# MooreThreads/LiteGS

Hardware: NVIDIA H100
Metric: forward+backward views/sec @1080p 1M Gaussians (higher is better)
Workload: dtype f32

## Files before the change

### litegs_b200/csrc/common.cuh

```cuda
#pragma once
#include <cuda_runtime.h>
#include <stdint.h>
#include <stdio.h>
#include <type_traits>

#define LGS_OK 0
#define LGS_ERR_ARG 10001
#define LGS_ERR_WORKSPACE 10002

void lgs_set_error(const char* fmt, ...);

#define LGS_REQUIRE(cond, ...)                                   \
    do {                                                         \
        if (!(cond)) {                                           \
            lgs_set_error(__VA_ARGS__);                          \
            return LGS_ERR_ARG;                                  \
        }                                                        \
    } while (0)

#define LGS_CHECK_LAUNCH(what)                                                               \
    do {                                                                                     \
        cudaError_t e__ = cudaGetLastError();                                                \
        if (e__ != cudaSuccess) {                                                            \
            lgs_set_error("%s: %s (%s:%d)", what, cudaGetErrorString(e__), __FILE__, __LINE__); \
// ... 12 lines not shown

static inline int lgs_cdiv(long long a, long long b) { return (int)((a + b - 1) / b); }
static inline bool lgs_tile_ok(int th, int tw)
{
    return (th == 8 && tw == 16) || (th == 12 && tw == 16) || (th == 16 && tw == 16) || (th == 8 && tw == 8);
}

template <typename F> static inline int lgs_with_flags(F&& f) { return f(); }
template <typename F, typename... R> static inline int lgs_with_flags(F&& f, bool b, R... rest)
{
    if (b) return lgs_with_flags([&](auto... c) { return f(std::true_type{}, c...); }, rest...);
    return lgs_with_flags([&](auto... c) { return f(std::false_type{}, c...); }, rest...);
}

template <typename F> static inline int lgs_with_tile(int th, int tw, F&& f)
{
    using I8 = std::integral_constant<int, 8>;
    using I12 = std::integral_constant<int, 12>;
    using I16 = std::integral_constant<int, 16>;
    if (th == 8 && tw == 16) return f(I8{}, I16{});
    if (th == 12 && tw == 16) return f(I12{}, I16{});
    if (th == 16 && tw == 16) return f(I16{}, I16{});
    return f(I8{}, I8{});
}

template <typename F> static inline int lgs_with_degree(int d, F&& f)
{
    switch (d) {
    case 0: return f(std::integral_constant<int, 0>{});
    case 1: return f(std::integral_constant<int, 1>{});
    case 2: return f(std::integral_constant<int, 2>{});
    default: return f(std::integral_constant<int, 3>{});
    }
}

template <auto K> static int lgs_max_threads()
{
    static const int n = [] { cudaFuncAttributes a; return cudaFuncGetAttributes(&a, K) == cudaSuccess ? a.maxThreadsPerBlock : 0; }();
    return n;
}

struct __align__(16) SplatRec {
    float px, py, A, B;
    float C, o, r, g;
    float b, depth, pad0, pad1;
};
static_assert(sizeof(SplatRec) == 48, "SplatRec must be 48 bytes");
#define LGS_REC_FLOATS 12

#define LGS_GRAD_FLOATS 12
#define LGS_GRAD_DEPTH 10
struct LgsRasterGrad { float dmx, dmy, dA, dB, dC, dop; };
#ifdef __CUDACC__
__device__ __forceinline__ void lgs_finish_raster_grad(const float4& a, const float4& c, const float4& e, float A, float B, float C,
                                                       float o, LgsRasterGrad& g)
{
    g.dmx = -(A * a.x + B * a.y);
    g.dmy = -(B * a.x + C * a.y);
    g.dA = -0.5f * a.z;
    g.dB = -a.w;
    g.dC = -0.5f * c.x;
    g.dop = (o > 0.0f) ? e.x / o : 0.0f;
}
#endif
```

### litegs_b200/csrc/raster.cu

```cuda
#include "common.cuh"

#define FULL_MASK 0xffffffffu
#define LOG2E 1.4426950408889634f
#define ALPHA_MIN (1.0f / 256.0f)
#define ALPHA_MAX (255.0f / 256.0f)
#define T_MIN (1.0f / 8192.0f)
#define WARPS_PER_BLOCK 4

__device__ __forceinline__ float fast_ex2(float x)
{
    float y;
    asm("ex2.approx.ftz.f32 %0, %1;" : "=f"(y) : "f"(x));
    return y;
}
__device__ __forceinline__ float fast_rcp(float x)
{
    float y;
    asm("rcp.approx.ftz.f32 %0, %1;" : "=f"(y) : "f"(x));
    return y;
}

__device__ __forceinline__ float2 add2(float2 a, float2 b) { return make_float2(__fadd_rn(a.x, b.x), __fadd_rn(a.y, b.y)); }
__device__ __forceinline__ float2 mul2(float2 a, float2 b) { return make_float2(__fmul_rn(a.x, b.x), __fmul_rn(a.y, b.y)); }
__device__ __forceinline__ float2 fma2(float2 a, float2 b, float2 c) { return make_float2(__fmaf_rn(a.x, b.x, c.x), __fmaf_rn(a.y, b.y, c.y)); }
// ... 31 lines not shown
        "@pk fma.rn.f32 %3, %9, w, %3;\n"
        "@pk fma.rn.f32 %4, %13, w, %4;\n"
        "@pk fma.rn.f32 %0, %12, w, %0;\n"
        "}\n"
        : "+f"(Ts), "+f"(Cr), "+f"(Cg), "+f"(Cb), "+f"(D), "+f"(nf)
        : "f"(a), "f"(cr), "f"(cg), "f"(cb), "f"(ts_min), "f"(a_min), "f"(neg_ki), "f"(z));
}
template <bool DEPTH>
__device__ __forceinline__ void blend_pixel_normal(float a, float cr, float cg, float cb, float z, float n0, float n1, float n2,
                                                   float& Ts, float& Cr, float& Cg, float& Cb, float& D, float& N0, float& N1,
                                                   float& N2, float& nf, float ts_min, float a_min, float neg_ki)
{
    if (DEPTH) {
        asm("{\n"
            ".reg .pred pa, pk;\n"
            ".reg .f32 w;\n"
            "setp.gt.f32 pa, %0, %13;\n"
            "@pa add.f32 %8, %8, 0f3F800000;\n"
            "setp.ge.and.f32 pk, %9, %14, pa;\n"
            "mul.f32 w, %9, %0;\n"
            "@pk fma.rn.f32 %1, %10, w, %1;\n"
            "@pk fma.rn.f32 %2, %11, w, %2;\n"
            "@pk fma.rn.f32 %3, %12, w, %3;\n"
            "@pk fma.rn.f32 %4, %16, w, %4;\n"
            "@pk fma.rn.f32 %5, %17, w, %5;\n"
            "@pk fma.rn.f32 %6, %18, w, %6;\n"
            "@pk fma.rn.f32 %7, %19, w, %7;\n"
            "@pk fma.rn.f32 %0, %15, w, %0;\n"
            "}\n"
            : "+f"(Ts), "+f"(Cr), "+f"(Cg), "+f"(Cb), "+f"(D), "+f"(N0), "+f"(N1), "+f"(N2), "+f"(nf)
            : "f"(a), "f"(cr), "f"(cg), "f"(cb), "f"(ts_min), "f"(a_min), "f"(neg_ki), "f"(z), "f"(n0), "f"(n1), "f"(n2));
    } else {
        asm("{\n"
            ".reg .pred pa, pk;\n"
            ".reg .f32 w;\n"
            "setp.gt.f32 pa, %0, %12;\n"
            "@pa add.f32 %7, %7, 0f3F800000;\n"
            "setp.ge.and.f32 pk, %8, %13, pa;\n"
            "mul.f32 w, %8, %0;\n"
            "@pk fma.rn.f32 %1, %9, w, %1;\n"
            "@pk fma.rn.f32 %2, %10, w, %2;\n"
            "@pk fma.rn.f32 %3, %11, w, %3;\n"
            "@pk fma.rn.f32 %4, %15, w, %4;\n"
            "@pk fma.rn.f32 %5, %16, w, %5;\n"
            "@pk fma.rn.f32 %6, %17, w, %6;\n"
            "@pk fma.rn.f32 %0, %14, w, %0;\n"
            "}\n"
            : "+f"(Ts), "+f"(Cr), "+f"(Cg), "+f"(Cb), "+f"(N0), "+f"(N1), "+f"(N2), "+f"(nf)
            : "f"(a), "f"(cr), "f"(cg), "f"(cb), "f"(ts_min), "f"(a_min), "f"(neg_ki), "f"(n0), "f"(n1), "f"(n2));
    }
    (void)z; (void)D;
}

__device__ __forceinline__ unsigned smem_u32(const void* p) { return (unsigned)__cvta_generic_to_shared(p); }
__device__ __forceinline__ void cp_async16(void* dst, const void* src)
{
    asm volatile("cp.async.cg.shared.global [%0], [%1], 16;\n" ::"r"(smem_u32(dst)), "l"(src));
}
__device__ __forceinline__ void cp_async_commit() { asm volatile("cp.async.commit_group;\n" ::); }
template <int N> __device__ __forceinline__ void cp_async_wait() { asm volatile("cp.async.wait_group %0;\n" ::"n"(N)); }

__device__ __forceinline__ void mbar_init(uint64_t* bar, unsigned count)
{
    asm volatile("mbarrier.init.shared::cta.b64 [%0], %1;\n" ::"r"(smem_u32(bar)), "r"(count));
}
__device__ __forceinline__ void mbar_expect_tx(uint64_t* bar, unsigned bytes)
{
    asm volatile("mbarrier.arrive.expect_tx.shared::cta.b64 _, [%0], %1;\n" ::"r"(smem_u32(bar)), "r"(bytes));
}
__device__ __forceinline__ bool mbar_try_wait(uint64_t* bar, unsigned parity)
{
    unsigned ok;
    asm volatile(
        "{\n"
        ".reg .pred p;\n"
        "mbarrier.try_wait.parity.shared::cta.b64 p, [%1], %2;\n"
        "selp.u32 %0, 1, 0, p;\n"
        "}\n"
        : "=r"(ok)
        : "r"(smem_u32(bar)), "r"(parity)
        : "memory");
    return ok != 0;
}
__device__ __forceinline__ void mbar_wait(uint64_t* bar, unsigned parity)
{
    while (!mbar_try_wait(bar, parity)) {}
}
__device__ __forceinline__ void bulk_g2s(void* dst, const void* src, unsigned bytes, uint64_t* bar)
{
    asm volatile("cp.async.bulk.shared::cluster.global.mbarrier::complete_tx::bytes [%0], [%1], %2, [%3];\n" ::"r"(smem_u32(dst)),
                 "l"(src), "r"(bytes), "r"(smem_u32(bar))
                 : "memory");
}

template <bool BULK>
struct Stager {
    SplatRec* buf;
    uint64_t* bar;
    unsigned phase_bits;
    unsigned pending;
    int lane;
    __device__ __forceinline__ void init(SplatRec* b, uint64_t* m, int ln)
    {
        buf = b; bar = m; lane = ln; phase_bits = 0; pending = 0;
        if (BULK) {
            if (lane == 0) { mbar_init(&bar[0], 1); mbar_init(&bar[1], 1); }
            asm volatile("fence.mbarrier_init.release.cluster;\n" ::);
            __syncwarp();
        }
    }
    template <bool NORMAL = false>
    __device__ __forceinline__ void issue(int which, const SplatRec* __restrict__ recs, int id, const float4* __restrict__ nrec = nullptr,
                                          float4* nbuf = nullptr)
// ... 957 lines not shown
```

### litegs_b200/csrc/sort.cu

```cuda
#include <cub/device/device_radix_sort.cuh>
#include <cub/block/block_scan.cuh>
#include <algorithm>
#include <cstdlib>
#include <cstring>
#include "common.cuh"

namespace {

constexpr int RS_THREADS = 256;
constexpr int RS_WARPS = RS_THREADS / 32;
constexpr int RS_MAXBINS = 256;

int g_sort_impl = -1;
bool g_sort_forced = false;

int sort_impl()
{
    if (g_sort_impl < 0) {
        const char* e = getenv("LGS_SORT");
        g_sort_forced = e != nullptr;
        g_sort_impl = (e != nullptr && strcmp(e, "cub") == 0) ? 0 : 1;
    }
    return g_sort_impl;
}
// ... 140 lines not shown
        for (int j = 0; j < NS; j++) {
            int r = s_cnt[w][d[j]];
#pragma unroll
            for (int q = 0; q < j; q++) r += __popc(mw[q * set_stride + d[j]]);
            own[j] = mw[j * set_stride + d[j]];
            rank[i0 + j] = (unsigned short)(r + __popc(own[j] & lt));
        }
        __syncwarp();
#pragma unroll
        for (int j = 0; j < NS; j++) {
            if ((own[j] >> lane) <= 1u) {
                if (NS == 1) s_cnt[w][d[j]] = (int)rank[i0 + j] + 1;
                else atomicAdd(&s_cnt[w][d[j]], __popc(own[j]));
                mw[j * set_stride + d[j]] = 0u;
            }
        }
        __syncwarp();
    }
    __syncthreads();
    int tot = 0;
#pragma unroll
    for (int k = 0; k < RS_WARPS; k++) { int c = s_cnt[k][t]; s_cnt[k][t] = tot; tot += c; }
    int dbase;
    BlockScan(s_scan).ExclusiveSum(tot, dbase);
#pragma unroll
    for (int k = 0; k < RS_WARPS; k++) s_cnt[k][t] += dbase;
    s_gofs[t] = gdig - dbase;
    __syncthreads();
#pragma unroll
    for (int i = 0; i < IPT; i++) {
        unsigned d = (((unsigned)key[i] - bias) >> shift) & mask;
        int p = s_cnt[w][d] + rank[i];
        s_k[p] = key[i];
        s_v[p] = val[i];
    }
    __syncthreads();
#pragma unroll
    for (int i = 0; i < IPT; i++) {
        int k = i * RS_THREADS + t;
        if (k < nvalid) {
            KeyT kk = s_k[k];
            int dst = s_gofs[(((unsigned)kk - bias) >> shift) & mask] + k;
            kout[dst] = kk;
            vout[dst] = s_v[k];
        }
    }
}

constexpr unsigned LB_AGG = 1u << 30, LB_INC = 2u << 30, LB_MASK = (1u << 30) - 1u;
constexpr int RS_MAXPASS = 4;

struct GhistArgs { int shift[RS_MAXPASS]; int nbins[RS_MAXPASS]; int passes; };

template <typename KeyT, int IPT>
__global__ void __launch_bounds__(RS_THREADS) rs_ghist_kernel(const KeyT* __restrict__ keys, int n, GhistArgs A, int* __restrict__ ghist,
                                                              unsigned bias, const int* __restrict__ n_dev,
                                                              const unsigned* __restrict__ bias_dev)
{
    constexpr int TILE = RS_THREADS * IPT;
    __shared__ int h[RS_MAXPASS][RS_MAXBINS];
    const int t = threadIdx.x;
    if (n_dev != nullptr) n = min(n, max(*n_dev, 0));
    if (bias_dev != nullptr) bias = *bias_dev;
    const int base = blockIdx.x * TILE;
    if (base >= n) return;
    for (int p = 0; p < A.passes; p++) h[p][t] = 0;
    __syncthreads();
#pragma unroll
    for (int i = 0; i < IPT; i++) {
        const int idx = base + i * RS_THREADS + t;
        if (idx < n) {
            const unsigned k = (unsigned)keys[idx] - bias;
            for (int p = 0; p < A.passes; p++) atomicAdd(&h[p][(k >> A.shift[p]) & (unsigned)(A.nbins[p] - 1)], 1);
        }
    }
    __syncthreads();
    for (int p = 0; p < A.passes; p++)
        if (t < A.nbins[p] && h[p][t] != 0) atomicAdd(&ghist[p * RS_MAXBINS + t], h[p][t]);
}

template <typename KeyT, int IPT>
__global__ void __launch_bounds__(RS_THREADS) rs_onesweep_kernel(const KeyT* __restrict__ kin, const unsigned* __restrict__ vin,
                                                                 KeyT* __restrict__ kout, unsigned* __restrict__ vout, int n, int shift,
                                                                 int nbins, const int* __restrict__ ghist ,
                                                                 unsigned* __restrict__ status ,
                                                                 int* __restrict__ ticket, unsigned bias, const int* __restrict__ n_dev,
                                                                 const unsigned* __restrict__ bias_dev)
{
    constexpr int TILE = RS_THREADS * IPT;
    using BlockScan = cub::BlockScan<int, RS_THREADS>;
    __shared__ int s_cnt[RS_WARPS][RS_MAXBINS];
    __shared__ int s_gofs[RS_MAXBINS];
    __shared__ KeyT s_k[TILE];
    __shared__ unsigned s_v[TILE];
    __shared__ int s_tile;
    static_assert(TILE >= RS_WARPS * RS_MAXBINS, "the match slots alias the value staging buffer");
    unsigned (*s_match)[RS_MAXBINS] = reinterpret_cast<unsigned (*)[RS_MAXBINS]>(s_v);
    __shared__ typename BlockScan::TempStorage s_scan;
    const int t = threadIdx.x, lane = t & 31, w = t >> 5;
    if (n_dev != nullptr) n = min(n, max(*n_dev, 0));
    if (bias_dev != nullptr) bias = *bias_dev;
    if (t == 0) s_tile = atomicAdd(ticket, 1);
#pragma unroll
    for (int k = 0; k < RS_WARPS; k++) { s_cnt[k][t] = 0; s_match[k][t] = 0u; }
    __syncthreads();
    const int tile = s_tile;
    const int base = tile * TILE;
    if (base >= n) return;
    const int nvalid = min(TILE, n - base);
    const unsigned mask = (unsigned)nbins - 1u;
    const unsigned lt = lanemask_lt();
    KeyT key[IPT];
    unsigned val[IPT];
    unsigned short rank[IPT];
#pragma unroll
    for (int i = 0; i < IPT; i++) {
        int loc = w * 32 * IPT + i * 32 + lane;
        bool valid = loc < nvalid;
        key[i] = valid ? kin[base + loc] : (KeyT)(bias - 1u);
        val[i] = valid ? vin[base + loc] : 0u;
    }
    int gdig;
    {
        int tot_d = t < nbins ? ghist[t] : 0;
        BlockScan(s_scan).ExclusiveSum(tot_d, gdig);
    }
    __syncthreads();
#pragma unroll
    for (int i = 0; i < IPT; i++) {
        unsigned d = (((unsigned)key[i] - bias) >> shift) & mask;
        atomicOr(&s_match[w][d], 1u << lane);
        __syncwarp();
        unsigned m = s_match[w][d];
        int r = s_cnt[w][d] + __popc(m & lt);
        rank[i] = (unsigned short)r;
        __syncwarp();
        if ((m >> lane) <= 1u) { s_cnt[w][d] = r + 1; s_match[w][d] = 0u; }
        __syncwarp();
    }
    __syncthreads();
    int tot = 0;
#pragma unroll
    for (int k = 0; k < RS_WARPS; k++) { int c = s_cnt[k][t]; s_cnt[k][t] = tot; tot += c; }
    int real = tot;
    if (t == (int)mask) real -= (TILE - nvalid);
    if (t < nbins) {
        volatile unsigned* st_ = status + (size_t)tile * nbins;
        st_[t] = LB_AGG | (unsigned)real;
        unsigned prefix = 0u;
        for (int i = tile - 1; i >= 0;) {
            const unsigned v = *((volatile unsigned*)(status + (size_t)i * nbins + t));
            const unsigned flag = v & ~LB_MASK;
            if (flag == 0u) continue;
            prefix += v & LB_MASK;
            if (flag == LB_INC) break;
            i--;
        }
        st_[t] = LB_INC | (prefix + (unsigned)real);
        gdig += (int)prefix;
    }
    int dbase;
    BlockScan(s_scan).ExclusiveSum(tot, dbase);
#pragma unroll
    for (int k = 0; k < RS_WARPS; k++) s_cnt[k][t] += dbase;
    s_gofs[t] = gdig - dbase;
    __syncthreads();
#pragma unroll
    for (int i = 0; i < IPT; i++) {
        unsigned d = (((unsigned)key[i] - bias) >> shift) & mask;
        int p = s_cnt[w][d] + rank[i];
        s_k[p] = key[i];
        s_v[p] = val[i];
    }
    __syncthreads();
#pragma unroll
    for (int i = 0; i < IPT; i++) {
        int k = i * RS_THREADS + t;
        if (k < nvalid) {
            KeyT kk = s_k[k];
            int dst = s_gofs[(((unsigned)kk - bias) >> shift) & mask] + k;
            kout[dst] = kk;
            vout[dst] = s_v[k];
        }
    }
}

struct RsPlan {
    int ipt, tile, nblocks, passes, dbits;
    size_t table_bytes, scan_bytes, total_bytes, off_scan, off_keys, off_vals;
};

inline size_t align256(size_t x) { return (x + 255) & ~(size_t)255; }

template <typename KeyT>
RsPlan rs_plan(int n, int begin_bit, int end_bit)
{
    RsPlan p;
    static const int forced_ipt = getenv("LGS_RS_IPT") ? atoi(getenv("LGS_RS_IPT")) : 0;
    p.ipt = (forced_ipt == 8 || forced_ipt == 16) ? forced_ipt : (n > (1 << 22) ? 16 : 8);
    p.tile = RS_THREADS * p.ipt;
    p.nblocks = (n + p.tile - 1) / p.tile;
    int bits = end_bit - begin_bit;
    p.passes = bits <= 0 ? 0 : (bits + 7) / 8;
    p.dbits = p.passes == 0 ? 0 : (bits + p.passes - 1) / p.passes;
    p.table_bytes = align256((size_t)RS_MAXPASS * RS_MAXBINS * p.nblocks * sizeof(int));
    p.scan_bytes = align256((RS_MAXPASS * RS_MAXBINS + 64) * sizeof(int));
    p.off_scan = p.table_bytes;
    p.off_keys = p.off_scan + p.scan_bytes;
    p.off_vals = p.off_keys + align256((size_t)n * sizeof(KeyT));
    p.total_bytes = p.off_vals + align256((size_t)n * sizeof(unsigned));
    return p;
}

bool rs_use_onesweep();
template <typename KeyT>
int rs_sort_onesweep(const KeyT* keys_in, KeyT* keys_out, const unsigned* vals_in, unsigned* vals_out, int n, int begin_bit, int end_bit,
                     unsigned bias, char* ws, cudaStream_t st, const int* n_dev, const unsigned* bias_dev);

template <typename KeyT>
int rs_sort(const KeyT* keys_in, KeyT* keys_out, const unsigned* vals_in, unsigned* vals_out, int n, int begin_bit, int end_bit,
            unsigned bias, char* ws, cudaStream_t st, const int* n_dev = nullptr, const unsigned* bias_dev = nullptr)
{
    RsPlan p = rs_plan<KeyT>(n, begin_bit, end_bit);
    if (p.passes == 0) {
        LGS_REQUIRE(n_dev == nullptr, "sort_pairs: a device-side count needs at least one pass");
        LGS_CUDA(cudaMemcpyAsync(keys_out, keys_in, (size_t)n * sizeof(KeyT), cudaMemcpyDeviceToDevice, st));
        LGS_CUDA(cudaMemcpyAsync(vals_out, vals_in, (size_t)n * sizeof(unsigned), cudaMemcpyDeviceToDevice, st));
        return LGS_OK;
    }
    if (rs_use_onesweep())
        return rs_sort_onesweep<KeyT>(keys_in, keys_out, vals_in, vals_out, n, begin_bit, end_bit, bias, ws, st, n_dev, bias_dev);
    int* table = (int*)ws;
    int* totals = (int*)(ws + p.off_scan);
    KeyT* ktmp = (KeyT*)(ws + p.off_keys);
    unsigned* vtmp = (unsigned*)(ws + p.off_vals);
    const KeyT* ksrc = keys_in;
    const unsigned* vsrc = vals_in;
    int bit = begin_bit;
    for (int pass = 0; pass < p.passes; pass++) {
        int dbits = min(p.dbits, end_bit - bit);
        int nbins = 1 << dbits;
        bool to_out = ((p.passes - 1 - pass) & 1) == 0;
        KeyT* kdst = to_out ? keys_out : ktmp;
        unsigned* vdst = to_out ? vals_out : vtmp;
        const bool vec = ((uintptr_t)ksrc & 15) == 0;
        lgs_with_flags([&](auto ipt16, auto v) {
            rs_hist_kernel<KeyT, ipt16 ? 16 : 8, v><<<p.nblocks, RS_THREADS, 0, st>>>(ksrc, n, bit, nbins, p.nblocks, table, bias, n_dev,
                                                                                     bias_dev);
            return LGS_OK;
        }, p.ipt == 16, vec);
        LGS_CHECK_LAUNCH("rs_hist_kernel");
        rs_scan_rows_kernel<<<nbins, RS_THREADS, 0, st>>>(table, p.nblocks, totals);
        LGS_CHECK_LAUNCH("rs_scan_rows_kernel");
        static const int rank_cap = getenv("LGS_RS_RANK") ? atoi(getenv("LGS_RS_RANK")) : 2;
        int ns = 1;
        while (ns < 4 && ns * 2 <= rank_cap && ns * 2 * RS_WARPS * nbins <= p.tile) ns *= 2;
        lgs_with_flags([&](auto ipt16, auto ns4, auto ns2) {
            rs_scatter_kernel<KeyT, ipt16 ? 16 : 8, ns4 ? 4 : ns2 ? 2 : 1><<<p.nblocks, RS_THREADS, 0, st>>>(
                ksrc, vsrc, kdst, vdst, n, bit, nbins, p.nblocks, table, totals, bias, n_dev, bias_dev);
            return LGS_OK;
        }, p.ipt == 16, ns == 4, ns == 2);
        LGS_CHECK_LAUNCH("rs_scatter_kernel");
        ksrc = kdst; vsrc = vdst;
        bit += dbits;
    }
    return LGS_OK;
}

int g_rs_onesweep = -1;
bool rs_use_onesweep()
{
    if (g_rs_onesweep < 0) {
        const char* e = getenv("LGS_RS");
        g_rs_onesweep = (e != nullptr && e[0] == 'o') ? 1 : 0;
    }
    return g_rs_onesweep == 1;
}

template <typename KeyT>
int rs_sort_onesweep(const KeyT* keys_in, KeyT* keys_out, const unsigned* vals_in, unsigned* vals_out, int n, int begin_bit, int end_bit,
                     unsigned bias, char* ws, cudaStream_t st, const int* n_dev, const unsigned* bias_dev)
{
    RsPlan p = rs_plan<KeyT>(n, begin_bit, end_bit);
    unsigned* status = (unsigned*)ws;
    int* ghist = (int*)(ws + p.off_scan);
    int* tickets = ghist + RS_MAXPASS * RS_MAXBINS;
    KeyT* ktmp = (KeyT*)(ws + p.off_keys);
    unsigned* vtmp = (unsigned*)(ws + p.off_vals);
    GhistArgs A;
    A.passes = p.passes;
    size_t status_words = 0;
    int bit = begin_bit;
    for (int pass = 0; pass < p.passes; pass++) {
        int dbits = min(p.dbits, end_bit - bit);
        A.shift[pass] = bit; A.nbins[pass] = 1 << dbits;
        status_words += (size_t)p.nblocks * A.nbins[pass];
        bit += dbits;
    }
    LGS_CUDA(cudaMemsetAsync(status, 0, status_words * sizeof(unsigned), st));
    LGS_CUDA(cudaMemsetAsync(ghist, 0, (RS_MAXPASS * RS_MAXBINS + 64) * sizeof(int), st));
    lgs_with_flags([&](auto ipt16) {
        rs_ghist_kernel<KeyT, ipt16 ? 16 : 8><<<p.nblocks, RS_THREADS, 0, st>>>(keys_in, n, A, ghist, bias, n_dev, bias_dev);
        return LGS_OK;
    }, p.ipt == 16);
    LGS_CHECK_LAUNCH("rs_ghist_kernel");
    const KeyT* ksrc = keys_in;
    const unsigned* vsrc = vals_in;
    size_t soff = 0;
    for (int pass = 0; pass < p.passes; pass++) {
        bool to_out = ((p.passes - 1 - pass) & 1) == 0;
        KeyT* kdst = to_out ? keys_out : ktmp;
        unsigned* vdst = to_out ? vals_out : vtmp;
        lgs_with_flags([&](auto ipt16) {
            rs_onesweep_kernel<KeyT, ipt16 ? 16 : 8><<<p.nblocks, RS_THREADS, 0, st>>>(ksrc, vsrc, kdst, vdst, n, A.shift[pass],
                A.nbins[pass], ghist + pass * RS_MAXBINS, status + soff, tickets + pass, bias, n_dev, bias_dev);
            return LGS_OK;
        }, p.ipt == 16);
        LGS_CHECK_LAUNCH("rs_onesweep_kernel");
        soff += (size_t)p.nblocks * A.nbins[pass];
        ksrc = kdst; vsrc = vdst;
    }
    return LGS_OK;
}

template <typename KeyT>
size_t sort_workspace_bytes(int n, int max_bits)
{
    size_t cubb = 0;
    cub::DeviceRadixSort::SortPairs<KeyT, unsigned>(nullptr, cubb, nullptr, nullptr, nullptr, nullptr, n, 0, max_bits);
    size_t own = rs_plan<KeyT>(n, 0, max_bits).total_bytes;
    return std::max(cubb, own) + 256;
}

template <typename KeyT>
int sort_pairs(const char* who, const KeyT* keys_in, KeyT* keys_out, const unsigned* vals_in, unsigned* vals_out, int n, int begin_bit,
               int end_bit, unsigned bias, void* workspace, size_t workspace_bytes, void* stream)
{
    if (n <= 0) return LGS_OK;
    LGS_REQUIRE(begin_bit >= 0 && end_bit >= begin_bit && end_bit <= (int)(8 * sizeof(KeyT)), "%s: bad bit range [%d, %d)", who, begin_bit,
                end_bit);
    char* ws = (char*)(((uintptr_t)workspace + 255) & ~(uintptr_t)255);
    size_t need;
    const int impl = sort_impl_for(n, end_bit - begin_bit, bias);
    if (impl == 0) {
        if (bias != 0u) { begin_bit = 0; end_bit = 8 * (int)sizeof(KeyT); }
        need = 0;
        cub::DeviceRadixSort::SortPairs<KeyT, unsigned>(nullptr, need, nullptr, nullptr, nullptr, nullptr, n, begin_bit, end_bit);
    } else {
        need = rs_plan<KeyT>(n, begin_bit, end_bit).total_bytes;
    }
    if (workspace == nullptr || workspace_bytes < need + 256) {
        lgs_set_error("%s: workspace of %zu bytes needed, %zu given", who, need + 256, workspace_bytes);
        return LGS_ERR_WORKSPACE;
    }
    if (impl == 0) {
        LGS_CUDA(cub::DeviceRadixSort::SortPairs<KeyT, unsigned>(ws, need, keys_in, keys_out, vals_in, vals_out, n, begin_bit, end_bit,
                                                                 (cudaStream_t)stream));
        return LGS_OK;
    }
    return rs_sort<KeyT>(keys_in, keys_out, vals_in, vals_out, n, begin_bit, end_bit, bias, ws, (cudaStream_t)stream);
}

}

extern "C" int lgs_set_sort_impl(int impl)
{
    LGS_REQUIRE(impl == -1 || impl == 0 || impl == 1, "set_sort_impl: %d is not -1 (unforced), 0 (cub) or 1 (lgs)", impl);
    g_sort_impl = impl;
    g_sort_forced = impl >= 0;
    return LGS_OK;
}

// ... 87 lines not shown
```

### profiles/microbench/dev_count_bench.py

```python
import ctypes
import sys, os
sys.path.insert(0, os.path.dirname(os.path.dirname(os.path.dirname(os.path.abspath(__file__)))))
import torch
from litegs_b200 import _lib

dev = torch.device("cuda:0")
st = lambda: torch.cuda.current_stream().cuda_stream
P = lambda t: t.data_ptr()


def timeit(fn, n=30):
    for _ in range(5):
        fn()
    torch.cuda.synchronize()
    e0 = torch.cuda.Event(enable_timing=True); e1 = torch.cuda.Event(enable_timing=True)
    e0.record()
    for _ in range(n):
        fn()
    e1.record(); torch.cuda.synchronize()
    return e0.elapsed_time(e1) / n * 1000.0


D = 10_897_674
for cap in (D, int(D * 1.3) + 65536):
    keys = torch.randint(1, 16201, (cap,), device=dev, dtype=torch.int32).to(torch.int16)
    vals = torch.arange(cap, device=dev, dtype=torch.int32)
    ko, vo = torch.empty_like(keys), torch.empty_like(vals)
    nb = ctypes.c_size_t(0)
    _lib.call("lgs_sort_pairs_u16_workspace_bytes", cap, ctypes.byref(nb))
    ws = torch.empty(nb.value, dtype=torch.uint8, device=dev)
    ndev = torch.tensor([D], dtype=torch.int32, device=dev)
    t_host = timeit(lambda: _lib.call("lgs_sort_pairs_u16", P(keys), P(ko), P(vals), P(vo), D, 0, 14, P(ws), ctypes.c_size_t(nb.value), st()))
    t_dev = timeit(lambda: _lib.call("lgs_sort_pairs_u16_dev", P(keys), P(ko), P(vals), P(vo), cap, P(ndev), 0, 14, P(ws), ctypes.c_size_t(nb.value), st()))
    print(f"tile sort D={D} capacity={cap}: host count {t_host:.1f} us, device count {t_dev:.1f} us")

N = 1_000_064
k32 = torch.randint(0, 1 << 24, (N,), device=dev, dtype=torch.int32)
v32 = torch.arange(N, device=dev, dtype=torch.int32)
ko, vo = torch.empty_like(k32), torch.empty_like(v32)
nb = ctypes.c_size_t(0)
_lib.call("lgs_sort_pairs_u32_workspace_bytes", N, ctypes.byref(nb))
ws = torch.empty(nb.value, dtype=torch.uint8, device=dev)
ndev = torch.tensor([984_960], dtype=torch.int32, device=dev)
bias = torch.zeros(1, dtype=torch.int32, device=dev)
t_host = timeit(lambda: _lib.call("lgs_sort_pairs_u32_rebased", P(k32), P(ko), P(v32), P(vo), 984_960, 0, 24, P(ws), ctypes.c_size_t(nb.value), st()))
t_dev = timeit(lambda: _lib.call("lgs_sort_pairs_u32_dev", P(k32), P(ko), P(v32), P(vo), N, P(ndev), P(bias), 24, P(ws), ctypes.c_size_t(nb.value), st()))
print(f"depth sort N=984960 (capacity {N}): host count {t_host:.1f} us, device count {t_dev:.1f} us")
cnt = torch.randint(0, 20, (N,), device=dev, dtype=torch.int32)
out = torch.empty(N, dtype=torch.int32, device=dev)
nb2 = ctypes.c_size_t(0)
_lib.call("lgs_scan_gathered_workspace_bytes", N, ctypes.byref(nb2))
ws2 = torch.empty(nb2.value, dtype=torch.uint8, device=dev)
order = torch.randperm(N, device=dev).to(torch.int32)
t_host = timeit(lambda: _lib.call("lgs_scan_gathered", P(cnt), P(order), 984_960, P(out), P(ws2), ctypes.c_size_t(nb2.value), st()))
t_dev = timeit(lambda: _lib.call("lgs_scan_gathered_dev", P(cnt), P(order), N, P(ndev), P(out), P(ws2), ctypes.c_size_t(nb2.value), st()))
print(f"gathered scan: host count {t_host:.1f} us, device count {t_dev:.1f} us")

D4 = 71_700_532
keys = torch.randint(1, 64801, (D4,), device=dev, dtype=torch.int32).to(torch.int16)
vals = torch.arange(D4, device=dev, dtype=torch.int32)
ko, vo = torch.empty_like(keys), torch.empty_like(vals)
nb = ctypes.c_size_t(0)
_lib.call("lgs_sort_pairs_u16_workspace_bytes", D4, ctypes.byref(nb))
ws = torch.empty(nb.value, dtype=torch.uint8, device=dev)
t = timeit(lambda: _lib.call("lgs_sort_pairs_u16", P(keys), P(ko), P(vals), P(vo), D4, 0, 16, P(ws), ctypes.c_size_t(nb.value), st()), n=10)
print(f"C4 tile sort D={D4}, 16 bits, LGS_RS_IPT={os.environ.get('LGS_RS_IPT', 'default')}, LGS_SORT={os.environ.get('LGS_SORT', 'lgs')}: {t:.1f} us "
      f"= {D4 * (2 + 2 * 12) / t / 1e6:.2f} TB/s of algorithmic traffic")
```

Baseline: 955.0.

## Rework onesweep radix sort with persistent tiles, cp.async staging, and windowed lookback

```diff
diff --git a/litegs_b200/csrc/common.cuh b/litegs_b200/csrc/common.cuh
--- a/litegs_b200/csrc/common.cuh
+++ b/litegs_b200/csrc/common.cuh
@@ -88,6 +88,14 @@
 #define LGS_GRAD_DEPTH 10
 struct LgsRasterGrad { float dmx, dmy, dA, dB, dC, dop; };
 #ifdef __CUDACC__
+__device__ __forceinline__ unsigned smem_u32(const void* p) { return (unsigned)__cvta_generic_to_shared(p); }
+__device__ __forceinline__ void cp_async16(void* dst, const void* src)
+{
+    asm volatile("cp.async.cg.shared.global [%0], [%1], 16;\n" ::"r"(smem_u32(dst)), "l"(src));
+}
+__device__ __forceinline__ void cp_async_commit() { asm volatile("cp.async.commit_group;\n" ::); }
+template <int N> __device__ __forceinline__ void cp_async_wait() { asm volatile("cp.async.wait_group %0;\n" ::"n"(N)); }
+
 __device__ __forceinline__ void lgs_finish_raster_grad(const float4& a, const float4& c, const float4& e, float A, float B, float C,
                                                        float o, LgsRasterGrad& g)
 {
diff --git a/litegs_b200/csrc/raster.cu b/litegs_b200/csrc/raster.cu
--- a/litegs_b200/csrc/raster.cu
+++ b/litegs_b200/csrc/raster.cu
@@ -107,13 +107,6 @@
     (void)z; (void)D;
 }
 
-__device__ __forceinline__ unsigned smem_u32(const void* p) { return (unsigned)__cvta_generic_to_shared(p); }
-__device__ __forceinline__ void cp_async16(void* dst, const void* src)
-{
-    asm volatile("cp.async.cg.shared.global [%0], [%1], 16;\n" ::"r"(smem_u32(dst)), "l"(src));
-}
-__device__ __forceinline__ void cp_async_commit() { asm volatile("cp.async.commit_group;\n" ::); }
-template <int N> __device__ __forceinline__ void cp_async_wait() { asm volatile("cp.async.wait_group %0;\n" ::"n"(N)); }
 
 __device__ __forceinline__ void mbar_init(uint64_t* bar, unsigned count)
 {
diff --git a/litegs_b200/csrc/sort.cu b/litegs_b200/csrc/sort.cu
--- a/litegs_b200/csrc/sort.cu
+++ b/litegs_b200/csrc/sort.cu
@@ -216,142 +216,212 @@
 
 struct GhistArgs { int shift[RS_MAXPASS]; int nbins[RS_MAXPASS]; int passes; };
 
-template <typename KeyT, int IPT>
+template <typename KeyT>
 __global__ void __launch_bounds__(RS_THREADS) rs_ghist_kernel(const KeyT* __restrict__ keys, int n, GhistArgs A, int* __restrict__ ghist,
                                                               unsigned bias, const int* __restrict__ n_dev,
                                                               const unsigned* __restrict__ bias_dev)
 {
-    constexpr int TILE = RS_THREADS * IPT;
+    constexpr int KPV = 16 / (int)sizeof(KeyT);
     __shared__ int h[RS_MAXPASS][RS_MAXBINS];
     const int t = threadIdx.x;
     if (n_dev != nullptr) n = min(n, max(*n_dev, 0));
     if (bias_dev != nullptr) bias = *bias_dev;
-    const int base = blockIdx.x * TILE;
-    if (base >= n) return;
-    for (int p = 0; p < A.passes; p++) h[p][t] = 0;
-    __syncthreads();
-#pragma unroll
-    for (int i = 0; i < IPT; i++) {
-        const int idx = base + i * RS_THREADS + t;
-        if (idx < n) {
-            const unsigned k = (unsigned)keys[idx] - bias;
-            for (int p = 0; p < A.passes; p++) atomicAdd(&h[p][(k >> A.shift[p]) & (unsigned)(A.nbins[p] - 1)], 1);
-        }
-    }
+#pragma unroll
+    for (int p = 0; p < RS_MAXPASS; p++) h[p][t] = 0;
+    __syncthreads();
+    auto count = [&](unsigned key) {
+        const unsigned k = key - bias;
+#pragma unroll
+        for (int p = 0; p < RS_MAXPASS; p++)
+            if (p < A.passes) atomicAdd(&h[p][(k >> A.shift[p]) & (unsigned)(A.nbins[p] - 1)], 1);
+    };
+    const int stride = gridDim.x * RS_THREADS;
+    int done = 0;
+    if (((uintptr_t)keys & 15) == 0) {
+        const int nv = n / KPV;
+        const uint4* v = reinterpret_cast<const uint4*>(keys);
+        for (int i = blockIdx.x * RS_THREADS + t; i < nv; i += stride) {
+            const uint4 q = v[i];
+            const unsigned x[4] = { q.x, q.y, q.z, q.w };
+#pragma unroll
+            for (int c = 0; c < 4; c++) {
+                if (sizeof(KeyT) == 2) { count(x[c] & 0xffffu); count(x[c] >> 16); }
+                else count(x[c]);
+            }
+        }
+        done = nv * KPV;
+    }
+    for (int i = done + blockIdx.x * RS_THREADS + t; i < n; i += stride) count((unsigned)keys[i]);
     __syncthreads();
     for (int p = 0; p < A.passes; p++)
         if (t < A.nbins[p] && h[p][t] != 0) atomicAdd(&ghist[p * RS_MAXBINS + t], h[p][t]);
 }
 
-template <typename KeyT, int IPT>
-__global__ void __launch_bounds__(RS_THREADS) rs_onesweep_kernel(const KeyT* __restrict__ kin, const unsigned* __restrict__ vin,
-                                                                 KeyT* __restrict__ kout, unsigned* __restrict__ vout, int n, int shift,
-                                                                 int nbins, const int* __restrict__ ghist ,
-                                                                 unsigned* __restrict__ status ,
-                                                                 int* __restrict__ ticket, unsigned bias, const int* __restrict__ n_dev,
-                                                                 const unsigned* __restrict__ bias_dev)
-{
-    constexpr int TILE = RS_THREADS * IPT;
-    using BlockScan = cub::BlockScan<int, RS_THREADS>;
-    __shared__ int s_cnt[RS_WARPS][RS_MAXBINS];
+constexpr int LB_WIN = 8;
+
+template <typename KeyT, int NT, int IPT>
+__global__ void __launch_bounds__(NT) rs_onesweep_kernel(const KeyT* __restrict__ kin, const unsigned* __restrict__ vin,
+                                                         KeyT* __restrict__ kout, unsigned* __restrict__ vout, int n, int shift,
+                                                         int nbins, const int* __restrict__ ghist ,
+                                                         unsigned* __restrict__ status ,
+                                                         int* __restrict__ ticket, unsigned bias, const int* __restrict__ n_dev,
+                                                         const unsigned* __restrict__ bias_dev)
+{
+    constexpr int NW = NT / 32, TILE = NT * IPT, NS = 2 * NW * RS_MAXBINS <= TILE ? 2 : 1;
+    static_assert(NT >= RS_MAXBINS, "thread t owns digit t in the block-wide steps");
+    static_assert(IPT % NS == 0 && NS * NW * RS_MAXBINS <= TILE, "the match slots of a round fit in the value staging buffer");
+    static_assert(TILE * sizeof(KeyT) % (16 * NT) == 0, "the staged keys are whole 16-byte copies of every thread");
+    using BlockScan = cub::BlockScan<int, NT>;
+    extern __shared__ __align__(16) unsigned char s_dyn[];
+    unsigned* s_v = reinterpret_cast<unsigned*>(s_dyn);
+    KeyT* s_k = reinterpret_cast<KeyT*>(s_v + TILE);
+    unsigned* s_match = s_v;
+    __shared__ int s_cnt[NW][RS_MAXBINS];
     __shared__ int s_gofs[RS_MAXBINS];
-    __shared__ KeyT s_k[TILE];
-    __shared__ unsigned s_v[TILE];
+    __shared__ int s_gdig[RS_MAXBINS];
+    __shared__ typename BlockScan::TempStorage s_scan;
     __shared__ int s_tile;
-    static_assert(TILE >= RS_WARPS * RS_MAXBINS, "the match slots alias the value staging buffer");
-    unsigned (*s_match)[RS_MAXBINS] = reinterpret_cast<unsigned (*)[RS_MAXBINS]>(s_v);
-    __shared__ typename BlockScan::TempStorage s_scan;
     const int t = threadIdx.x, lane = t & 31, w = t >> 5;
     if (n_dev != nullptr) n = min(n, max(*n_dev, 0));
     if (bias_dev != nullptr) bias = *bias_dev;
-    if (t == 0) s_tile = atomicAdd(ticket, 1);
-#pragma unroll
-    for (int k = 0; k < RS_WARPS; k++) { s_cnt[k][t] = 0; s_match[k][t] = 0u; }
-    __syncthreads();
-    const int tile = s_tile;
-    const int base = tile * TILE;
-    if (base >= n) return;
-    const int nvalid = min(TILE, n - base);
     const unsigned mask = (unsigned)nbins - 1u;
     const unsigned lt = lanemask_lt();
-    KeyT key[IPT];
-    unsigned val[IPT];
-    unsigned short rank[IPT];
-#pragma unroll
-    for (int i = 0; i < IPT; i++) {
-        int loc = w * 32 * IPT + i * 32 + lane;
-        bool valid = loc < nvalid;
-        key[i] = valid ? kin[base + loc] : (KeyT)(bias - 1u);
-        val[i] = valid ? vin[base + loc] : 0u;
-    }
-    int gdig;
+    const bool aligned = (((uintptr_t)kin | (uintptr_t)vin) & 15) == 0;
     {
-        int tot_d = t < nbins ? ghist[t] : 0;
-        BlockScan(s_scan).ExclusiveSum(tot_d, gdig);
-    }
-    __syncthreads();
-#pragma unroll
-    for (int i = 0; i < IPT; i++) {
-        unsigned d = (((unsigned)key[i] - bias) >> shift) & mask;
-        atomicOr(&s_match[w][d], 1u << lane);
-        __syncwarp();
-        unsigned m = s_match[w][d];
-        int r = s_cnt[w][d] + __popc(m & lt);
-        rank[i] = (unsigned short)r;
-        __syncwarp();
-        if ((m >> lane) <= 1u) { s_cnt[w][d] = r + 1; s_match[w][d] = 0u; }
-        __syncwarp();
-    }
-    __syncthreads();
-    int tot = 0;
-#pragma unroll
-    for (int k = 0; k < RS_WARPS; k++) { int c = s_cnt[k][t]; s_cnt[k][t] = tot; tot += c; }
-    int real = tot;
-    if (t == (int)mask) real -= (TILE - nvalid);
-    if (t < nbins) {
-        volatile unsigned* st_ = status + (size_t)tile * nbins;
-        st_[t] = LB_AGG | (unsigned)real;
-        unsigned prefix = 0u;
-        for (int i = tile - 1; i >= 0;) {
-            const unsigned v = *((volatile unsigned*)(status + (size_t)i * nbins + t));
-            const unsigned flag = v & ~LB_MASK;
-            if (flag == 0u) continue;
-            prefix += v & LB_MASK;
-            if (flag == LB_INC) break;
-            i--;
-        }
-        st_[t] = LB_INC | (prefix + (unsigned)real);
-        gdig += (int)prefix;
-    }
-    int dbase;
-    BlockScan(s_scan).ExclusiveSum(tot, dbase);
-#pragma unroll
-    for (int k = 0; k < RS_WARPS; k++) s_cnt[k][t] += dbase;
-    s_gofs[t] = gdig - dbase;
-    __syncthreads();
-#pragma unroll
-    for (int i = 0; i < IPT; i++) {
-        unsigned d = (((unsigned)key[i] - bias) >> shift) & mask;
-        int p = s_cnt[w][d] + rank[i];
-        s_k[p] = key[i];
-        s_v[p] = val[i];
-    }
-    __syncthreads();
-#pragma unroll
-    for (int i = 0; i < IPT; i++) {
-        int k = i * RS_THREADS + t;
-        if (k < nvalid) {
-            KeyT kk = s_k[k];
-            int dst = s_gofs[(((unsigned)kk - bias) >> shift) & mask] + k;
-            kout[dst] = kk;
-            vout[dst] = s_v[k];
-        }
+        int g;
+        BlockScan(s_scan).ExclusiveSum(t < nbins ? ghist[t] : 0, g);
+        if (t < RS_MAXBINS) s_gdig[t] = g;
+    }
+    if (t == 0) s_tile = atomicAdd(ticket, 1);
+    __syncthreads();
+    for (int tile = s_tile; (long long)tile * TILE < n; tile = s_tile) {
+        const int base = tile * TILE;
+        const int nvalid = min(TILE, n - base);
+        const bool staged = aligned && nvalid == TILE;
+        if (staged) {
+            const char* gv = reinterpret_cast<const char*>(vin + base);
+            const char* gk = reinterpret_cast<const char*>(kin + base);
+            for (int c = t * 16; c < TILE * 4; c += NT * 16) cp_async16(s_dyn + c, gv + c);
+            for (int c = t * 16; c < TILE * (int)sizeof(KeyT); c += NT * 16) cp_async16(s_dyn + TILE * 4 + c, gk + c);
+            cp_async_commit();
+            cp_async_wait<0>();
+            __syncthreads();
+        }
+        KeyT key[IPT];
+        unsigned val[IPT];
+        unsigned short rank[IPT];
+#pragma unroll
+        for (int i = 0; i < IPT; i++) {
+            int loc = w * 32 * IPT + i * 32 + lane;
+            if (staged) {
+                key[i] = s_k[loc];
+                val[i] = s_v[loc];
+            } else {
+                bool valid = loc < nvalid;
+                key[i] = valid ? kin[base + loc] : (KeyT)(bias - 1u);
+                val[i] = valid ? vin[base + loc] : 0u;
+            }
+        }
+        if (staged) __syncthreads();
+        for (int k = t; k < NW * RS_MAXBINS; k += NT) (&s_cnt[0][0])[k] = 0;
+        for (int k = t; k < NS * NW * nbins; k += NT) s_match[k] = 0u;
+        __syncthreads();
+        unsigned* mw = s_match + w * nbins;
+        const int set_stride = NW * nbins;
+#pragma unroll
+        for (int i0 = 0; i0 < IPT; i0 += NS) {
+            unsigned d[NS];
+#pragma unroll
+            for (int q = 0; q < NS; q++) {
+                d[q] = (((unsigned)key[i0 + q] - bias) >> shift) & mask;
+                atomicOr(&mw[q * set_stride + d[q]], 1u << lane);
+            }
+            __syncwarp();
+            unsigned own[NS];
+#pragma unroll
+            for (int j = 0; j < NS; j++) {
+                int r = s_cnt[w][d[j]];
+#pragma unroll
+                for (int q = 0; q < j; q++) r += __popc(mw[q * set_stride + d[j]]);
+                own[j] = mw[j * set_stride + d[j]];
+                rank[i0 + j] = (unsigned short)(r + __popc(own[j] & lt));
+            }
+            __syncwarp();
+#pragma unroll
+            for (int j = 0; j < NS; j++) {
+                if ((own[j] >> lane) <= 1u) {
+                    atomicAdd(&s_cnt[w][d[j]], __popc(own[j]));
+                    mw[j * set_stride + d[j]] = 0u;
+                }
+            }
+            __syncwarp();
+        }
+        __syncthreads();
+        int tot = 0;
+        if (t < RS_MAXBINS) {
+#pragma unroll
+            for (int k = 0; k < NW; k++) { int c = s_cnt[k][t]; s_cnt[k][t] = tot; tot += c; }
+        }
+        unsigned* st_ = status + (size_t)tile * nbins;
+        int real = 0;
+        if (t < nbins) {
+            real = tot - (t == (int)mask ? TILE - nvalid : 0);
+            *((volatile unsigned*)&st_[t]) = (tile == 0 ? LB_INC : LB_AGG) | (unsigned)real;
+        }
+        int dbase;
+        BlockScan(s_scan).ExclusiveSum(tot, dbase);
+        if (t < RS_MAXBINS) {
+#pragma unroll
+            for (int k = 0; k < NW; k++) s_cnt[k][t] += dbase;
+        }
+        __syncthreads();
+#pragma unroll
+        for (int i = 0; i < IPT; i++) {
+            unsigned d = (((unsigned)key[i] - bias) >> shift) & mask;
+            int p = s_cnt[w][d] + rank[i];
+            s_k[p] = key[i];
+            s_v[p] = val[i];
+        }
+        if (t < nbins) {
+            unsigned prefix = 0u;
+            for (int j = tile - 1; j >= 0;) {
+                unsigned v[LB_WIN];
+#pragma unroll
+                for (int k = 0; k < LB_WIN; k++)
+                    v[k] = j - k >= 0 ? *((const volatile unsigned*)&status[(size_t)(j - k) * nbins + t]) : LB_INC;
+                int used = 0;
+                bool inc = false;
+#pragma unroll
+                for (int k = 0; k < LB_WIN; k++) {
+                    const unsigned flag = v[k] & ~LB_MASK;
+                    if (used == k && !inc && flag != 0u) { prefix += v[k] & LB_MASK; used++; inc = flag == LB_INC; }
+                }
+                if (inc) break;
+                if (used == 0) __nanosleep(256);
+                j -= used;
+            }
+            if (tile > 0) *((volatile unsigned*)&st_[t]) = LB_INC | (prefix + (unsigned)real);
+            s_gofs[t] = s_gdig[t] + (int)prefix - dbase;
+        }
+        __syncthreads();
+#pragma unroll
+        for (int i = 0; i < IPT; i++) {
+            int k = i * NT + t;
+            if (k < nvalid) {
+                KeyT kk = s_k[k];
+                int dst = s_gofs[(((unsigned)kk - bias) >> shift) & mask] + k;
+                kout[dst] = kk;
+                vout[dst] = s_v[k];
+            }
+        }
+        if (t == 0) s_tile = atomicAdd(ticket, 1);
+        __syncthreads();
     }
 }
 
 struct RsPlan {
     int ipt, tile, nblocks, passes, dbits;
-    size_t table_bytes, scan_bytes, total_bytes, off_scan, off_keys, off_vals;
+    size_t table_bytes, scan_bytes, total_bytes, off_scan, off_table, off_keys, off_vals;
 };
 
 inline size_t align256(size_t x) { return (x + 255) & ~(size_t)255; }
@@ -360,8 +430,7 @@
 RsPlan rs_plan(int n, int begin_bit, int end_bit)
 {
     RsPlan p;
-    static const int forced_ipt = getenv("LGS_RS_IPT") ? atoi(getenv("LGS_RS_IPT")) : 0;
-    p.ipt = (forced_ipt == 8 || forced_ipt == 16) ? forced_ipt : (n > (1 << 22) ? 16 : 8);
+    p.ipt = n > (1 << 22) ? 16 : 8;
     p.tile = RS_THREADS * p.ipt;
     p.nblocks = (n + p.tile - 1) / p.tile;
     int bits = end_bit - begin_bit;
@@ -369,8 +438,9 @@
     p.dbits = p.passes == 0 ? 0 : (bits + p.passes - 1) / p.passes;
     p.table_bytes = align256((size_t)RS_MAXPASS * RS_MAXBINS * p.nblocks * sizeof(int));
     p.scan_bytes = align256((RS_MAXPASS * RS_MAXBINS + 64) * sizeof(int));
-    p.off_scan = p.table_bytes;
-    p.off_keys = p.off_scan + p.scan_bytes;
+    p.off_scan = 0;
+    p.off_table = p.scan_bytes;
+    p.off_keys = p.off_table + p.table_bytes;
     p.off_vals = p.off_keys + align256((size_t)n * sizeof(KeyT));
     p.total_bytes = p.off_vals + align256((size_t)n * sizeof(unsigned));
     return p;
@@ -394,7 +464,7 @@
     }
     if (rs_use_onesweep())
         return rs_sort_onesweep<KeyT>(keys_in, keys_out, vals_in, vals_out, n, begin_bit, end_bit, bias, ws, st, n_dev, bias_dev);
-    int* table = (int*)ws;
+    int* table = (int*)(ws + p.off_table);
     int* totals = (int*)(ws + p.off_scan);
     KeyT* ktmp = (KeyT*)(ws + p.off_keys);
     unsigned* vtmp = (unsigned*)(ws + p.off_vals);
@@ -416,14 +486,12 @@
         LGS_CHECK_LAUNCH("rs_hist_kernel");
         rs_scan_rows_kernel<<<nbins, RS_THREADS, 0, st>>>(table, p.nblocks, totals);
         LGS_CHECK_LAUNCH("rs_scan_rows_kernel");
-        static const int rank_cap = getenv("LGS_RS_RANK") ? atoi(getenv("LGS_RS_RANK")) : 2;
-        int ns = 1;
-        while (ns < 4 && ns * 2 <= rank_cap && ns * 2 * RS_WARPS * nbins <= p.tile) ns *= 2;
-        lgs_with_flags([&](auto ipt16, auto ns4, auto ns2) {
-            rs_scatter_kernel<KeyT, ipt16 ? 16 : 8, ns4 ? 4 : ns2 ? 2 : 1><<<p.nblocks, RS_THREADS, 0, st>>>(
+        const bool ns2 = 2 * RS_WARPS * nbins <= p.tile;
+        lgs_with_flags([&](auto ipt16, auto two) {
+            rs_scatter_kernel<KeyT, ipt16 ? 16 : 8, two ? 2 : 1><<<p.nblocks, RS_THREADS, 0, st>>>(
                 ksrc, vsrc, kdst, vdst, n, bit, nbins, p.nblocks, table, totals, bias, n_dev, bias_dev);
             return LGS_OK;
-        }, p.ipt == 16, ns == 4, ns == 2);
+        }, p.ipt == 16, ns2);
         LGS_CHECK_LAUNCH("rs_scatter_kernel");
         ksrc = kdst; vsrc = vdst;
         bit += dbits;
@@ -436,19 +504,46 @@
 {
     if (g_rs_onesweep < 0) {
         const char* e = getenv("LGS_RS");
-        g_rs_onesweep = (e != nullptr && e[0] == 'o') ? 1 : 0;
+        g_rs_onesweep = (e != nullptr && e[0] == 'p') ? 0 : 1;
     }
     return g_rs_onesweep == 1;
 }
+
+template <typename KeyT, int NT, int IPT>
+int rs_onesweep_pass(const KeyT* ksrc, const unsigned* vsrc, KeyT* kdst, unsigned* vdst, int n, int shift, int nbins, const int* ghist,
+                     unsigned* status, int* ticket, unsigned bias, cudaStream_t st, const int* n_dev, const unsigned* bias_dev, int sms)
+{
+    constexpr int TILE = NT * IPT;
+    constexpr int smem = TILE * (int)(sizeof(unsigned) + sizeof(KeyT));
+    auto kern = rs_onesweep_kernel<KeyT, NT, IPT>;
+    static const int resident = [&] {
+        int b = 0;
+        if (cudaFuncSetAttribute(kern, cudaFuncAttributeMaxDynamicSharedMemorySize, smem) != cudaSuccess ||
+            cudaOccupancyMaxActiveBlocksPerMultiprocessor(&b, kern, NT, smem) != cudaSuccess) return 0;
+        return b;
+    }();
+    LGS_REQUIRE(resident > 0, "rs_onesweep_kernel: no CTA of %d threads and %d bytes of shared memory fits an SM", NT, smem);
+    const int grid = std::min((n + TILE - 1) / TILE, resident * sms);
+    kern<<<grid, NT, smem, st>>>(ksrc, vsrc, kdst, vdst, n, shift, nbins, ghist, status, ticket, bias, n_dev, bias_dev);
+    LGS_CHECK_LAUNCH("rs_onesweep_kernel");
+    return LGS_OK;
+}
+
+template <typename KeyT> struct RsOnesweepShape { static constexpr int NT = 256, IPT = 16; };
+template <> struct RsOnesweepShape<unsigned short> { static constexpr int NT = 512, IPT = 24; };
+
+
 
 template <typename KeyT>
 int rs_sort_onesweep(const KeyT* keys_in, KeyT* keys_out, const unsigned* vals_in, unsigned* vals_out, int n, int begin_bit, int end_bit,
                      unsigned bias, char* ws, cudaStream_t st, const int* n_dev, const unsigned* bias_dev)
 {
     RsPlan p = rs_plan<KeyT>(n, begin_bit, end_bit);
-    unsigned* status = (unsigned*)ws;
+    using S = RsOnesweepShape<KeyT>;
+    const int ntiles = (n + S::NT * S::IPT - 1) / (S::NT * S::IPT);
     int* ghist = (int*)(ws + p.off_scan);
     int* tickets = ghist + RS_MAXPASS * RS_MAXBINS;
+    unsigned* status = (unsigned*)(ws + p.off_table);
     KeyT* ktmp = (KeyT*)(ws + p.off_keys);
     unsigned* vtmp = (unsigned*)(ws + p.off_vals);
     GhistArgs A;
@@ -458,15 +553,15 @@
     for (int pass = 0; pass < p.passes; pass++) {
         int dbits = min(p.dbits, end_bit - bit);
         A.shift[pass] = bit; A.nbins[pass] = 1 << dbits;
-        status_words += (size_t)p.nblocks * A.nbins[pass];
+        status_words += (size_t)ntiles * A.nbins[pass];
         bit += dbits;
     }
-    LGS_CUDA(cudaMemsetAsync(status, 0, status_words * sizeof(unsigned), st));
-    LGS_CUDA(cudaMemsetAsync(ghist, 0, (RS_MAXPASS * RS_MAXBINS + 64) * sizeof(int), st));
-    lgs_with_flags([&](auto ipt16) {
-        rs_ghist_kernel<KeyT, ipt16 ? 16 : 8><<<p.nblocks, RS_THREADS, 0, st>>>(keys_in, n, A, ghist, bias, n_dev, bias_dev);
-        return LGS_OK;
-    }, p.ipt == 16);
+    LGS_CUDA(cudaMemsetAsync(ws, 0, p.off_table + status_words * sizeof(unsigned), st));
+    int dev = 0, sms = 0;
+    LGS_CUDA(cudaGetDevice(&dev));
+    LGS_CUDA(cudaDeviceGetAttribute(&sms, cudaDevAttrMultiProcessorCount, dev));
+    rs_ghist_kernel<KeyT><<<std::min((n + RS_THREADS * 16 - 1) / (RS_THREADS * 16), 8 * sms), RS_THREADS, 0, st>>>(keys_in, n, A, ghist,
+                                                                                                                   bias, n_dev, bias_dev);
     LGS_CHECK_LAUNCH("rs_ghist_kernel");
     const KeyT* ksrc = keys_in;
     const unsigned* vsrc = vals_in;
@@ -475,13 +570,11 @@
         bool to_out = ((p.passes - 1 - pass) & 1) == 0;
         KeyT* kdst = to_out ? keys_out : ktmp;
         unsigned* vdst = to_out ? vals_out : vtmp;
-        lgs_with_flags([&](auto ipt16) {
-            rs_onesweep_kernel<KeyT, ipt16 ? 16 : 8><<<p.nblocks, RS_THREADS, 0, st>>>(ksrc, vsrc, kdst, vdst, n, A.shift[pass],
-                A.nbins[pass], ghist + pass * RS_MAXBINS, status + soff, tickets + pass, bias, n_dev, bias_dev);
-            return LGS_OK;
-        }, p.ipt == 16);
-        LGS_CHECK_LAUNCH("rs_onesweep_kernel");
-        soff += (size_t)p.nblocks * A.nbins[pass];
+        const int rc = rs_onesweep_pass<KeyT, S::NT, S::IPT>(ksrc, vsrc, kdst, vdst, n, A.shift[pass], A.nbins[pass],
+                                                             ghist + pass * RS_MAXBINS, status + soff, tickets + pass, bias, st, n_dev,
+                                                             bias_dev, sms);
+        if (rc != LGS_OK) return rc;
+        soff += (size_t)ntiles * A.nbins[pass];
         ksrc = kdst; vsrc = vdst;
     }
     return LGS_OK;
diff --git a/profiles/microbench/binning_bench.py b/profiles/microbench/binning_bench.py
--- /dev/null
+++ b/profiles/microbench/binning_bench.py
@@ -0,0 +1,160 @@
+import argparse
+import ctypes
+import json
+import os
+import subprocess
+import sys
+
+sys.path.insert(0, os.path.dirname(os.path.dirname(os.path.dirname(os.path.abspath(__file__)))))
+import torch
+
+from litegs_b200 import _lib, pipeline, scene
+from litegs_b200.dist import PARAM_ORDER
+
+ap = argparse.ArgumentParser()
+ap.add_argument("--out", default=None, metavar="DIR", help="also write the results to DIR/binning_bench.json")
+ap.add_argument("--iters", type=int, default=50)
+ap.add_argument("--no-c4", action="store_true")
+args = ap.parse_args()
+
+dev = torch.device("cuda:0")
+P = lambda t: ctypes.c_void_p(t.data_ptr())
+st = lambda: ctypes.c_void_p(torch.cuda.current_stream().cuda_stream)
+FORMS = {"passes": 0, "onesweep": 1}
+
+
+def card():
+    try:
+        q = subprocess.run(["nvidia-smi", "--query-gpu=name,power.limit,clocks.max.sm", "--format=csv,noheader"], capture_output=True,
+                           text=True, timeout=30).stdout.strip().splitlines()[0]
+    except Exception as e:
+        q = f"nvidia-smi unavailable: {e}"
+    return f"{torch.cuda.get_device_name(0)} | {q}"
+
+
+def timeit(fn, n):
+    for _ in range(5):
+        fn()
+    torch.cuda.synchronize()
+    e0, e1 = torch.cuda.Event(enable_timing=True), torch.cuda.Event(enable_timing=True)
+    e0.record()
+    for _ in range(n):
+        fn()
+    e1.record()
+    torch.cuda.synchronize()
+    return e0.elapsed_time(e1) / n * 1e3
+
+
+def kernel_split(fn, calls=5):
+    fn(); torch.cuda.synchronize()
+    with torch.profiler.profile(activities=[torch.profiler.ProfilerActivity.CUDA]) as prof:
+        for _ in range(calls):
+            fn()
+        torch.cuda.synchronize()
+    out = {}
+    for ev in prof.key_averages():
+        t = getattr(ev, "device_time_total", None)
+        if t is None:
+            t = ev.cuda_time_total
+        if t > 0:
+            out[ev.key[:90]] = round(t / calls, 2)
+    return dict(sorted(out.items(), key=lambda kv: -kv[1]))
+
+
+def copy_ceiling(nbytes):
+    a = torch.empty(nbytes, dtype=torch.uint8, device=dev)
+    b = torch.empty_like(a)
+    return timeit(lambda: b.copy_(a), args.iters)
+
+
+W, H, tile = 1920, 1080, (8, 16)
+p = scene.make_scene(1_000_000, sh_degree=3, seed=0, log_scale_range=(0.002, 0.02))
+Pt = {k: torch.from_numpy(p[k]).to(dev) for k in PARAM_ORDER}
+A = [torch.from_numpy(p[k]).to(dev) for k in ("cluster_origin", "cluster_extend")]
+cam = {k: torch.from_numpy(v).to(dev) for k, v in scene.make_camera(0, 64, W, H).items()}
+pairs, bits = pipeline.probe_view_sizes(Pt, A[0], A[1], [cam], 3, (H, W), tile)
+cap, planned = int(pairs * 1.3) + 65536, min(32, 8 * ((bits + 7) // 8))
+ws = pipeline.ViewWorkspace(Pt, (H, W), tile, cap, planned, use_graphs=False)
+side = torch.cuda.Stream(device=dev)
+with torch.cuda.stream(side):
+    ws.forward(Pt, A[0], A[1], cam, 3)
+torch.cuda.synchronize()
+vparams = ws.vparams.clone()
+vp = vparams.cpu()
+n_live, d_live, bias = int(vp[0]), int(vp[1]), int(vp[2]) & 0xFFFFFFFF
+assert d_live == pairs, (d_live, pairs)
+tkeys, tvals = ws.keys.clone(), ws.vals.clone()
+dkeys, dvals = ws.dkey.clone(), ws.iota.clone()
+N, D, tbits = ws.Nmax, ws.cap, ws.ntile.bit_length()
+info = {"card": card(), "D_live": d_live, "D_capacity": D, "tile_bits": tbits, "N_live": n_live, "N_capacity": N,
+        "depth_bits": planned, "depth_bias": bias}
+print(json.dumps(info))
+del ws
+torch.cuda.empty_cache()
+
+res = {"info": info, "tile": {}, "depth": {}}
+nb = ctypes.c_size_t(0)
+_lib.call("lgs_sort_pairs_u16_workspace_bytes", D, ctypes.byref(nb))
+tws, tnb = torch.empty(nb.value, dtype=torch.uint8, device=dev), ctypes.c_size_t(nb.value)
+_lib.call("lgs_sort_pairs_u32_workspace_bytes", N, ctypes.byref(nb))
+dws, dnb = torch.empty(nb.value, dtype=torch.uint8, device=dev), ctypes.c_size_t(nb.value)
+tko, tvo = torch.empty_like(tkeys), torch.empty_like(tvals)
+dko, dvo = torch.empty_like(dkeys), torch.empty_like(dvals)
+n_dev, d_dev, b_dev = (vparams[i:i + 1].clone() for i in range(3))
+
+tile_sort = lambda: _lib.call("lgs_sort_pairs_u16_dev", P(tkeys), P(tko), P(tvals), P(tvo), D, P(d_dev), 0, tbits, P(tws), tnb, st())
+depth_sort = lambda: _lib.call("lgs_sort_pairs_u32_dev", P(dkeys), P(dko), P(dvals), P(dvo), N, P(n_dev), P(b_dev), planned, P(dws), dnb,
+                               st())
+
+ref = {}
+for form, f in FORMS.items():
+    _lib.call("lgs_set_radix_form", f)
+    for name, fn, nbytes in (("tile", tile_sort, 26 * d_live), ("depth", depth_sort, 68 * n_live)):
+        us = timeit(fn, args.iters)
+        out = (tko[:d_live].clone(), tvo[:d_live].clone()) if name == "tile" else (dko[:n_live].clone(), dvo[:n_live].clone())
+        if name in ref:
+            same = all(torch.equal(a, b) for a, b in zip(ref[name], out))
+        else:
+            ref[name], same = out, True
+        res[name][form] = {"us": round(us, 1), "TB/s": round(nbytes / us / 1e6, 3), "same_as_passes": same,
+                           "kernels_us": kernel_split(fn)}
+        print(f"{name} sort, {form}: {us:.1f} us = {nbytes / us / 1e6:.2f} TB/s of algorithmic traffic; bit-equal to passes: {same}")
+        for k, v in res[name][form]["kernels_us"].items():
+            print(f"    {v:9.2f} us  {k}")
+_lib.call("lgs_set_sort_impl", 0)
+cub_us = timeit(lambda: _lib.call("lgs_sort_pairs_u16", P(tkeys), P(tko), P(tvals), P(tvo), d_live, 0, tbits, P(tws), tnb, st()), args.iters)
+_lib.call("lgs_set_sort_impl", -1)
+res["tile"]["cub_host_count"] = {"us": round(cub_us, 1), "TB/s": round(26 * d_live / cub_us / 1e6, 3)}
+print(f"tile sort, cub (host count): {cub_us:.1f} us")
+
+for name, nbytes in (("tile", 26 * d_live), ("depth", 68 * n_live)):
+    us = copy_ceiling(nbytes // 2)
+    res[name]["copy_ceiling"] = {"us": round(us, 1), "TB/s": round(nbytes / us / 1e6, 3)}
+    print(f"{name}: device-to-device copy of {nbytes // 2} bytes (same traffic): {us:.1f} us = {nbytes / us / 1e6:.2f} TB/s")
+
+if not args.no_c4:
+    del tkeys, tvals, tko, tvo, tws
+    torch.cuda.empty_cache()
+    D4 = 71_700_532
+    g = torch.Generator(device="cpu").manual_seed(4)
+    start = torch.randint(1, 64801 - 6, (D4 // 7 + 1,), generator=g, dtype=torch.int32)
+    k4 = (start[:, None] + torch.arange(7, dtype=torch.int32)[None, :]).reshape(-1)[:D4].to(torch.int16).to(dev)
+    v4 = torch.arange(D4, dtype=torch.int32, device=dev)
+    ko4, vo4 = torch.empty_like(k4), torch.empty_like(v4)
+    _lib.call("lgs_sort_pairs_u16_workspace_bytes", D4, ctypes.byref(nb))
+    ws4, nb4 = torch.empty(nb.value, dtype=torch.uint8, device=dev), ctypes.c_size_t(nb.value)
+    c4 = {}
+    for impl, (si, form) in {"own_passes": (1, 0), "own_onesweep": (1, 1), "cub": (0, 0)}.items():
+        _lib.call("lgs_set_sort_impl", si)
+        _lib.call("lgs_set_radix_form", form)
+        us = timeit(lambda: _lib.call("lgs_sort_pairs_u16", P(k4), P(ko4), P(v4), P(vo4), D4, 0, 16, P(ws4), nb4, st()), 10)
+        c4[impl] = {"us": round(us, 1), "TB/s": round(26 * D4 / us / 1e6, 3)}
+        print(f"C4 tile sort shape ({D4} pairs, 16 bits, host count), {impl}: {us:.1f} us = {26 * D4 / us / 1e6:.2f} TB/s")
+    _lib.call("lgs_set_sort_impl", -1)
+    res["c4_tile_sort"] = c4
+
+print(info["card"])
+if args.out is not None:
+    os.makedirs(args.out, exist_ok=True)
+    with open(os.path.join(args.out, "binning_bench.json"), "w") as f:
+        json.dump(res, f, indent=1)
diff --git a/profiles/microbench/dev_count_bench.py b/profiles/microbench/dev_count_bench.py
--- a/profiles/microbench/dev_count_bench.py
+++ b/profiles/microbench/dev_count_bench.py
@@ -64,5 +64,5 @@
 _lib.call("lgs_sort_pairs_u16_workspace_bytes", D4, ctypes.byref(nb))
 ws = torch.empty(nb.value, dtype=torch.uint8, device=dev)
 t = timeit(lambda: _lib.call("lgs_sort_pairs_u16", P(keys), P(ko), P(vals), P(vo), D4, 0, 16, P(ws), ctypes.c_size_t(nb.value), st()), n=10)
-print(f"C4 tile sort D={D4}, 16 bits, LGS_RS_IPT={os.environ.get('LGS_RS_IPT', 'default')}, LGS_SORT={os.environ.get('LGS_SORT', 'lgs')}: {t:.1f} us "
+print(f"C4 tile sort D={D4}, 16 bits, LGS_SORT={os.environ.get('LGS_SORT', 'lgs')}: {t:.1f} us "
       f"= {D4 * (2 + 2 * 12) / t / 1e6:.2f} TB/s of algorithmic traffic")
```

Measured after the change: 976.6 (median of 6 runs). 1.02x the previous value.
